# Tomeu7/AO-MARL

Measured on AMD Instinct MI355X. Metric: env steps/sec (AO frames/sec), higher is better.
Workload: dtype f32

## Files before the change

### ao_marl_amd/csrc/aomarl_capi.hip

```cpp
#include "aomarl_kernels.hip"

#include <math.h>
#include <stdlib.h>
#include <stdarg.h>
#include <stdio.h>
#include <string.h>

#include <algorithm>
#include <climits>
#include <string>
#include <vector>

static thread_local char g_err[512] = "";

int fail(const char *fmt, ...) {
  va_list ap;
  va_start(ap, fmt);
  vsnprintf(g_err, sizeof(g_err), fmt, ap);
  va_end(ap);
  return 1;
}


struct aomarl_ctx {
// ... 19 lines not shown
  bool small_ok = false;
  int reset_streams = 2;
  bool reset_prefetch_whole = true;
  hipEvent_t ev_reset = nullptr, ev_reset2[3] = {nullptr, nullptr, nullptr};
  bool no_extrude_sg = false;
  bool defer_dm_shape = false;
  int fused_debug = 0;
  bool prefetch_atmos = false, premoved = false;
  bool frame_wait_pending = false;
  bool screens_dirty_main = true;
  float cmat_scale = 1.f, v2m_scale = 1.f, m2v_scale = 1.f, s2m_scale = 1.f, ab_scale[AOMARL_MAX_LAYERS] = {1.f, 1.f, 1.f, 1.f, 1.f, 1.f, 1.f, 1.f};
  bool subpixel_flow = false;
  float frac_x[AOMARL_MAX_LAYERS] = {0, 0, 0, 0, 0, 0, 0, 0}, frac_y[AOMARL_MAX_LAYERS] = {0, 0, 0, 0, 0, 0, 0, 0};
  bool graph_step = false, capturing = false, side_joined = false, fork_recorded = false;
  hipEvent_t ev_fork = nullptr;
  struct StepGraph { std::vector<long long> key; hipGraphExec_t exec; hipGraph_t graph; unsigned long long arith[AR_N]; int fw_variant[6]; };
  std::vector<StepGraph> graphs;
  unsigned long long graph_hits = 0, graph_captures = 0;
  unsigned long long cfg_epoch = 0;
  const int32_t *sel_checked = nullptr;
  int sel_checked_n = 0, sel_checked_nm = 0;
  int fw_variant[6] = {0, 0, 0, 0, 0, 0};
  char fw_name[96] = {0};
  bool time_fw = false;
  std::vector<hipEvent_t> fw_ev;
  size_t fw_ev_used = 0;
  std::vector<hipEvent_t> fw_ev_retired;
  hipStream_t atm_stream = nullptr, psf_stream = nullptr;
  hipEvent_t ev_frame = nullptr, ev_moved = nullptr, ev_psf = nullptr;
  hipEvent_t ev_frame_cur = nullptr;
  bool frame_marked = false;
  struct FramePipe {
    bool have_twin = false, active = false;
    const float *owner_screens = nullptr;
    aomarl_state twin;
    int par = 0;
    hipStream_t fstream = nullptr;
    hipEvent_t ev_cmd = nullptr, ev_commit = nullptr, ev_done[2] = {nullptr, nullptr}, ev_psf[2] = {nullptr, nullptr};
    hipEvent_t ev_done_cur[2] = {nullptr, nullptr};
    bool psf_out[2] = {false, false};
    bool cmd_covers_commit = false;
    bool cmd_covers_psf = false;
    int32_t *snap[2] = {nullptr, nullptr};
    size_t snap_ints = 0;
    unsigned long long steps = 0, overlapped = 0, behind = 0;
  } pipe;
// ... 737 lines not shown
```

### ao_marl_amd/csrc/aomarl_capi_composites.hip

```cpp
const char *aomarl_frame_kernel_name(aomarl_ctx *c) {
  if (!c || !c->fw_variant[0]) return "";
  snprintf(c->fw_name, sizeof(c->fw_name), "k_frame_wave<%d, %d, %s, %s, %s, %s>", c->fw_variant[0], c->fw_variant[1],
           c->fw_variant[2] ? "true" : "false", c->fw_variant[3] ? "true" : "false",
           c->fw_variant[4] ? "true" : "false", c->fw_variant[5] ? "true" : "false");
  return c->fw_name;
}

int aomarl_frame_kernel_time(aomarl_ctx *c, double *total_ms, int *launches) {
  if (!c || !total_ms || !launches) return fail("frame_kernel_time: null argument");
  double tot = 0.0;
  int n = 0;
  for (size_t i = 0; i + 1 < c->fw_ev_used; i += 2) {
    float ms = 0.f;
    HIPCHK(hipEventSynchronize(c->fw_ev[i + 1]));
    HIPCHK(hipEventElapsedTime(&ms, c->fw_ev[i], c->fw_ev[i + 1]));
    tot += ms; n++;
  }
  { const int rrc = fw_ev_rewind(c); if (rrc) return rrc; }
  *total_ms = tot; *launches = n;
  return 0;
}

int aomarl_frame_fused_available(aomarl_ctx *c) {
  return c && c->sys.fused_ok && !c->force_unfused_frame ? 1 : 0;
}

static int frame_fused_impl(aomarl_ctx *c, aomarl_state *st, int b, int n, int flags, void *stream, int slot);

int aomarl_frame_fused(aomarl_ctx *c, aomarl_state *st, int b, int n, int flags, void *stream) {
  return frame_fused_impl(c, st, b, n, flags, stream, -1);
}

static int frame_fused_impl(aomarl_ctx *c, aomarl_state *st, int b, int n, int flags, void *stream, int slot) {
  int rc = check_range(c, st, b, n);
  if (rc) return rc;
  if (slot < 0) {
    rc = atmos_wait_pending(c, stream);
    if (rc) return rc;
    rc = psf_wait_pending(c, stream);
    if (rc) return rc;
  }
  if (!c->sys.fused_ok) return fail("frame_fused: geometry not eligible (see aomarl_frame_fused_available)");
  if (flags & (AOMARL_IMG_FROM_PHASE_BUFFER | AOMARL_IMG_NO_ATMOS | AOMARL_IMG_NO_DMS))
    return fail("frame_fused: FROM_PHASE_BUFFER / NO_ATMOS / NO_DMS are not supported here");
  const bool noise = (flags & AOMARL_IMG_NOISE) && c->sys.noise >= 0.f;
  const bool cube = flags & AOMARL_IMG_WRITE_BINCUBE;
  const bool otf = flags & AOMARL_IMG_DM_FROM_VOLTAGE;
  const int cog = ((flags & AOMARL_IMG_COG) ? 1 : 0) | (c->fused_debug << 8);
  if (otf && !c->sys.otf_ok) return fail("frame_fused: DM_FROM_VOLTAGE needs a separable stack-array lattice (see aomarl_dm_from_voltage_available)");
  if (cube && !st->bincube) return fail("frame_fused: WRITE_BINCUBE needs st->bincube");
  if (!cube && !(cog & 1)) return fail("frame_fused: nothing to produce (neither bincube nor slopes)");
  if (n == 0) return 0;
  hipStream_t s = (hipStream_t)stream;
  Work w = work_layout(c, st->nenv);
  const int W = 2 * c->sys.hw;
  float *TR = st->work + w.TR + (size_t)b * c->sys.pupdiam * W * 2;
  float *TP = st->work + w.TPART + (size_t)b * w.nblk * 4;
  float *PEND = st->work + w.PEND + (size_t)b * (W * W + 4);
  DevState ds = dev_state(st);
  if (w.nblk != c->sys.ntiles) return fail("frame_fused: internal stripe count mismatch");
  const int nb = otf ? c->sys.otf_nb : 1;
  const bool hp = c->dft_mode < 0 ? g_precision != 0 : c->dft_mode == 1;
  const bool qf = FW_QF && otf && !hp && !noise && !cube;
  const bool dma = FW_DMA && otf && (hp || FW_DMA_F32);
  const size_t smm = sizeof(float) * ((qf ? 0 : 2 * 128) + (otf ? 4 * 4 * nb * c->sys.otf_latw : 0)) + FW_SLOT_BYTES(dma) +
                     (dma ? 4 * FWD_WAVE(c->nlayers == 1 ? 1 : 3) : 128) +
                     (qf ? 4 * 16 * (size_t)c->sys.ntiles : 0);
  static const long lds_pad_env = [] { const char *e = getenv("AOMARL_FW_LDS_PAD"); return e ? atol(e) : -1L; }();
  size_t lds_pad = 0;
  if (qf && slot >= 0 && smm >= 40 * 1024) {
    const size_t two_per_cu = (160 * 1024) / 3 + 64;
    lds_pad = lds_pad_env >= 0 ? (size_t)lds_pad_env : (smm < two_per_cu ? (two_per_cu - smm + 63) / 64 * 64 : 0);
    if (smm + lds_pad > 64 * 1024) lds_pad = 0;
  }
  dim3 grid((n + 3) / 4, c->sys.ntiles), blk(256);
#define FW(NL, NB, OTF, NZ, WC, HP) hipExtLaunchKernelGGL((k_frame_wave<NL, NB, OTF, NZ, WC, HP>), grid, blk, smm + lds_pad, s, ev_start, ev_done, 0, c->sys, ds, b, n, cog, TR, TP, w.nblk)
#define FW_H(NL, NB, OTF, NZ, WC) do { if (hp) FW(NL, NB, OTF, NZ, WC, true); else FW(NL, NB, OTF, NZ, WC, false); } while (0)
#define FW_NC(NL, NB, OTF)                                                                     \
  do {                                                                                          \
    if (noise) { if (cube) FW_H(NL, NB, OTF, true, true); else FW_H(NL, NB, OTF, true, false); }     \
    else { if (cube) FW_H(NL, NB, OTF, false, true); else FW_H(NL, NB, OTF, false, false); }         \
  } while (0)
#define FW_L(NL)                                                          \
  do {                                                                    \
    if (!otf) FW_NC(NL, 1, false);                                        \
    else if (nb == 1) FW_NC(NL, 1, true);                                 \
    else FW_NC(NL, 2, true);                                              \
  } while (0)
  const bool timed = !c->capturing && c->time_fw && c->fw_ev_used + 2 <= c->fw_ev.size();
  hipEvent_t ev_start = nullptr, ev_done = nullptr;
  if (c->prefetch_atmos) {
    rc = side_stream(c);
    if (rc) return rc;
    ev_done = slot < 0 ? c->ev_frame : c->pipe.ev_done[slot];
  }
  if (timed) { ev_start = c->fw_ev[c->fw_ev_used]; ev_done = c->fw_ev[c->fw_ev_used + 1]; c->fw_ev_used += 2; }
  hipEvent_t ev_mark = nullptr;
  if (c->capturing) { ev_mark = ev_done; ev_start = nullptr; ev_done = nullptr; }
// ... 198 lines not shown
```

### ao_marl_amd/csrc/aomarl_capi_stages.hip

```cpp
static int dm_shape_impl(aomarl_ctx *c, aomarl_state *st, int b, int n, const float *volts,
                         bool skip_stack, void *stream) {
  const float *v = volts ? volts : st->voltage + (size_t)b * st->ld_actu;
  const int ldv = volts ? c->sys.nactu : st->ld_actu;
  DevState ds = dev_state(st);
  for (int k = 0; k < c->ndm; k++) {
    const DevDm &D = c->sys.dms[k];
    const int np = D.dim * D.dim;
    if (D.type == AOMARL_DM_TT)
      hipLaunchKernelGGL(k_dm_shape, dim3(1, n), dim3(64), 0, (hipStream_t)stream, c->sys, ds, b, k, v, ldv);
    else if (skip_stack)
      continue;
    else if (D.sep && !c->force_generic_dm)
      hipLaunchKernelGGL(k_dm_shape_sep, dim3((D.dim + DMS_TX - 1) / DMS_TX, (D.dim + DMS_TY - 1) / DMS_TY, n),
                         dim3(256), 0, (hipStream_t)stream, c->sys, ds, b, k, v, ldv);
    else
      hipLaunchKernelGGL(k_dm_shape, dim3((np + 255) / 256, n), dim3(256), 0, (hipStream_t)stream, c->sys, ds, b, k, v, ldv);
    LAUNCHCHK();
  }
  return 0;
}

int aomarl_comp_dm_shape(aomarl_ctx *c, aomarl_state *st, int b, int n, const float *volts, void *stream) {
  int rc = check_range(c, st, b, n);
  if (rc) return rc;
// ... 52 lines not shown
  if (!strcmp(name, "residual_shortcut")) {
    if (value && (!c->s2m || c->s2m_nmodes < 1)) return fail("residual_shortcut: no v2m . cmat matrix (aomarl_set_slopes2modes)");
    c->residual_shortcut = value != 0;
    return 0;
  }
  if (!strcmp(name, "reset_streams")) { c->reset_streams = value < 1 ? 1 : (value > 4 ? 4 : value); return 0; }
  if (!strcmp(name, "reset_prefetch_whole")) { c->reset_prefetch_whole = value != 0; return 0; }
  if (!strcmp(name, "extrude_unfused")) { c->no_extrude_sg = value != 0; return 0; }
  if (!strcmp(name, "reset_untransposed")) { c->reset_untransposed = value != 0; return 0; }
  if (!strcmp(name, "time_frame_kernel")) {
    c->time_fw = value > 0;
    { const int rrc = fw_ev_rewind(c); if (rrc) return rrc; }
    while (c->fw_ev.size() < 2 * (size_t)std::max(value, 0)) {
      hipEvent_t e;
      HIPCHK(hipEventCreate(&e));
      c->fw_ev.push_back(e);
    }
    return 0;
  }
  if (!strcmp(name, "prefetch_atmos")) { c->prefetch_atmos = value != 0; return 0; }
  if (!strcmp(name, "subpixel_flow")) { c->subpixel_flow = value != 0; return 0; }
  if (!strcmp(name, "graph_step")) { c->graph_step = value != 0; return 0; }
  if (!strcmp(name, "fused_debug")) { c->fused_debug = value; return 0; }
  if (!strcmp(name, "force_f32_dft")) { c->dft_mode = value < 0 ? -1 : (value != 0 ? 0 : 1); return 0; }
  if (!strcmp(name, "force_unfused_frame")) { c->force_unfused_frame = value != 0; return 0; }
  if (!strcmp(name, "force_generic_spot")) { c->force_generic_spot = value != 0; return 0; }
  if (!strcmp(name, "force_generic_target")) { c->force_generic_target = value != 0; return 0; }
  return fail("set_option: unknown option %s", name);
}

static DevSys traced_sys(const aomarl_ctx *c) {
  DevSys sy = c->sys;
  if (c->subpixel_flow)
    for (int l = 0; l < c->nlayers; l++) {
      sy.layers[l].wxo += c->frac_x[l]; sy.layers[l].txo += c->frac_x[l];
      sy.layers[l].wyo += c->frac_y[l]; sy.layers[l].tyo += c->frac_y[l];
    }
  return sy;
}

int aomarl_raytrace_wfs(aomarl_ctx *c, aomarl_state *st, int b, int n, int flags, void *stream) {
  int rc = check_range(c, st, b, n);
  if (rc) return rc;
  rc = atmos_wait_pending(c, stream);
  if (rc) return rc;
  if (!st->wfs_phase) return fail("raytrace_wfs needs st->wfs_phase");
// ... 350 lines not shown
```

### ao_marl_amd/csrc/aomarl_kernels.hip

```cpp
#include "aomarl_host.h"
#include "aomarl_gemm_p.h"
#include <type_traits>

#define WAVE 64

typedef unsigned u32x4 __attribute__((ext_vector_type(4)));

__device__ __forceinline__ hx2 cvt_h2(float a, float b) {
  return __builtin_bit_cast(hx2, __builtin_amdgcn_cvt_pkrtz(a, b));
}
__device__ __forceinline__ float sub_lo(hx2 h, float a) {
  float r;
  asm("v_fma_mix_f32 %0, %1, -1.0, %2 op_sel_hi:[1,0,0]" : "=v"(r) : "v"(h), "v"(a));
  return r;
}
__device__ __forceinline__ float sub_hi(hx2 h, float a) {
  float r;
  asm("v_fma_mix_f32 %0, %1, -1.0, %2 op_sel:[1,0,0] op_sel_hi:[1,0,0]" : "=v"(r) : "v"(h), "v"(a));
  return r;
}

struct __attribute__((packed, aligned(4))) f4u { float v[4]; };
__device__ __forceinline__ void add4(float acc[4], const float *p) {
  const f4u t = *reinterpret_cast<const f4u *>(p);
// ... 2088 lines not shown
#endif
#define FW_SLOT_BYTES(dma) ((dma) ? (FW_SLOTS1 ? 2 * 3 * 1024 : 16384) : 16384)
#define FWD_BLK 1152
#define FWD_IMG (2 * 1024 + 128)
#define FWD_WAVE(nl) ((nl) * FWD_IMG)
__global__ __launch_bounds__(256) __attribute__((amdgpu_waves_per_eu(FW_WAVES, FW_WAVES)))
void k_frame_wave(DevSys sys, DevState st, int env_begin,
                                                    int env_count, int do_cog,
                                                    float *__restrict__ TR,
                                                    float *__restrict__ TPART, int nblk) {
  extern __shared__ float smem[];
  const int pd = sys.pupdiam, ntl = sys.ntiles;
  const int tid = threadIdx.x, lane = tid & 63, q = lane >> 4, c = lane & 15;
  const int wv = __builtin_amdgcn_readfirstlane(tid >> 6);
  constexpr bool QF = FW_QF && OTF && !HP && !NOISE && !WRITE_CUBE;
  constexpr bool DMA = FW_DMA && OTF && (HP || FW_DMA_F32);
  float2 *sTw = reinterpret_cast<float2 *>(smem);
  float *lat_all = reinterpret_cast<float *>(sTw + (QF ? 0 : 128));
  float4 *shb = reinterpret_cast<float4 *>(lat_all + 4 * 4 * NB * (OTF ? sys.otf_latw : 0));
  char *dimg = reinterpret_cast<char *>(shb) + FW_SLOT_BYTES(DMA) + (DMA ? wv * FWD_WAVE(NL) : 0);
  float4 *qmom = reinterpret_cast<float4 *>(reinterpret_cast<char *>(shb) + FW_SLOT_BYTES(DMA) + (DMA ? 4 * FWD_WAVE(NL) : 0)) + wv * ntl;
  const int dbg = do_cog >> 8;
  do_cog &= 1;
  const int r = sys.stripe_order[blockIdx.y];
  const int el = 4 * blockIdx.x + wv;
  if constexpr (!QF) {
    if (tid < 128) {
      float sn, cs;
      sincospif((float)tid * (1.0f / 64.0f), &sn, &cs);
      sTw[tid] = make_float2(cs, sn);
    }
    __syncthreads();
  }
  const bool active = el < env_count;
  const int e = env_begin + (active ? el : env_count - 1);
  float Cc[4] = {0.f, 0.f, 0.f, 0.f}, Ss[4] = {0.f, 0.f, 0.f, 0.f};
  if constexpr (!QF) {
#pragma unroll
    for (int s = 0; s < 4; s++) {
      const float2 w = sTw[((4 * q + s) * (2 * c + 1)) & 127];
      Cc[s] = w.x; Ss[s] = w.y;
    }
  }
  SpotTwH twh;
  if (HP) twh = spot_tw_h(Cc, Ss);
  SpotQf qfk;
  if constexpr (QF) {
    const float4 ka = reinterpret_cast<const float4 *>(sys.qf_tab)[2 * lane], kb = reinterpret_cast<const float4 *>(sys.qf_tab)[2 * lane + 1];
    qfk.Ml = f32x2{ka.x, ka.y}; qfk.Mh = f32x2{ka.z, ka.w};
    qfk.Sl = f32x2{kb.x, kb.y}; qfk.Sh = f32x2{kb.z, kb.w};
  }
  unsigned shstep;
  const int y = 16 * r + c;
  const char *layb[NL];
  __amdgpu_buffer_rsrc_t lrs[NL];
  unsigned lpxs[NL], ldim[NL], lvo[NL];
#pragma unroll
  for (int l = 0; l < NL; l++) {
    const DevLayer &L = sys.layers[l];
    layb[l] = reinterpret_cast<const char *>(st.screens + (long long)e * sys.screen_stride + L.screen_off);
    lrs[l] = __builtin_amdgcn_make_buffer_rsrc(const_cast<char *>(layb[l]), 0,
                                               4 * L.dim * (L.dim + RING_PAD), 0x00020000);
    ldim[l] = (unsigned)L.dim;
    int px = L.tox + st.origin[(e * sys.nlayers + l) * 2]; px -= (px >= L.dim) ? L.dim : 0;
    int py = L.toy + st.origin[(e * sys.nlayers + l) * 2 + 1]; py -= (py >= L.dim) ? L.dim : 0;
    lpxs[l] = (unsigned)px;
    unsigned pr = (unsigned)y + (unsigned)py; pr = min(pr, pr - ldim[l]);
    lvo[l] = 4u * (pr * (ldim[l] + RING_PAD) + 4u * (unsigned)q);
  }
  const DevDm &D0 = sys.dms[0], &D1 = sys.dms[1];
  const float *pzt = st.dm_shape + (long long)e * sys.shape_stride + D0.shape_off;
  const float *ttslot = st.dm_shape + (long long)e * sys.shape_stride + D1.shape_off;
  const float c0 = ttslot[0], c1 = ttslot[1];
  const int half = pd / 2;
  const unsigned pvo = 4u * ((unsigned)(y + D0.toy) * (unsigned)D0.dim + (unsigned)D0.tox + 4u * (unsigned)q);
  const unsigned tvo = 32u * ((unsigned)y * (unsigned)(pd >> 2) + (unsigned)q);
  const unsigned mvo = 2u * (unsigned)y * (unsigned)ntl;
  const char *pztb = reinterpret_cast<const char *>(pzt);
  const char *ttb = reinterpret_cast<const char *>(sys.tt_pk);
  const char *mkb = reinterpret_cast<const char *>(sys.tile_mask);
  const bool sh_tt = wv < 2;
  const void *shbase = sh_tt ? static_cast<const void *>(ttb) : (HP ? sys.psf_tw_h : sys.psf_tw_f);
  const __amdgpu_buffer_rsrc_t shrs = __builtin_amdgcn_make_buffer_rsrc(
      const_cast<void *>(shbase), 0, sh_tt ? 8 * pd * pd : ntl * 1024, 0x00020000);
  const unsigned shvo = sh_tt ? tvo + 16u * (unsigned)wv : 16u * (unsigned)lane;
  shstep = sh_tt ? 7u : 10u;
  float pivot;
  {
    float v = OTF ? ttslot[2] : pzt[(half + D0.toy) * D0.dim + half + D0.tox];
    const float2 f = reinterpret_cast<const float2 *>(D1.influ)[(half + D1.toy) * D1.dim + half + D1.tox];
    v += c0 * f.x + c1 * f.y;
#pragma unroll
    for (int l = 0; l < NL; l++) {
      const DevLayer &L = sys.layers[l];
      int py = L.toy + st.origin[(e * sys.nlayers + l) * 2 + 1]; py -= (py >= L.dim) ? L.dim : 0;
      unsigned pyc = (unsigned)(half + py); pyc = min(pyc, pyc - ldim[l]);
      unsigned pxc = (unsigned)half + lpxs[l]; pxc = min(pxc, pxc - ldim[l]);
      v += reinterpret_cast<const float *>(layb[l])[pyc * (ldim[l] + RING_PAD) + pxc];
    }
    pivot = v;
  }
  float Pxr[NB], Pyr[NB];
  const int jm = (c >> 2) + 4 * (c & 3);
  const bool jm_ok = jm < 4 * NB;
  const int latw = sys.otf_latw, tpn = sys.otf_tpn;
  float *lat = lat_all + wv * (4 * NB * latw);
  if (OTF) {
#pragma unroll
    for (int s = 0; s < NB; s++) {
      const int ax = sys.otf_xoff + c - D0.pitch * (q + 4 * s);
      const int ay = sys.otf_yoff + c - D0.pitch * (q + 4 * s);
      Pxr[s] = (ax >= 0 && ax < D0.ss) ? D0.prof[ax] : 0.f;
      Pyr[s] = (ay >= 0 && ay < D0.ss) ? D0.prof[ay] : 0.f;
    }
    const float *volt = st.voltage + (long long)e * st.ld_actu + D0.com_off;
    for (int i = 0; i < 4 * NB; i++) {
      const int gy = sys.otf_gy0 + r * tpn + i;
      for (int jj = lane; jj < latw; jj += 64) {
        const int gx = sys.otf_gx0 + jj;
        float v = 0.f;
        if (gx >= 0 && gx < D0.gw && gy >= 0 && gy < D0.gh) {
          const int a = D0.grid[gy * D0.gw + gx];
          if (a >= 0) v = volt[a];
        }
        lat[i * latw + jj] = v;
      }
    }
    __builtin_amdgcn_wave_barrier();
  }
  const float *latq = lat + (jm_ok ? jm : 0);
  const float wfs_il = sys.wfs_inv_lambda, tar_il = sys.tar_inv_lambda;
  const f32x4 Z4 = opaque_zero4();
  f32x4 PA = {0.f, 0.f, 0.f, 0.f}, PB = {0.f, 0.f, 0.f, 0.f};
  float R0r = 0.f, R0i = 0.f;
  float sd = 0.f, sd2 = 0.f, sm = 0.f;
  int nlit = 0;
  constexpr bool PK = OTF && !HP;
  const f32x4 NP4 = {-pivot, -pivot, -pivot, -pivot};
  const f32x2 c0c0 = {c0, c0}, c1c1 = {c1, c1};
  const f32x2 wil2 = {sys.wfs_inv_lambda, sys.wfs_inv_lambda}, til2 = {sys.tar_inv_lambda, sys.tar_inv_lambda};
  f32x2 sdp = {0.f, 0.f}, sd2p = {0.f, 0.f}, R0rp = {0.f, 0.f}, R0ip = {0.f, 0.f};
  int nfull = 0;

  const const_float_p cflux = (const_float_p)(unsigned long long)sys.flux;
  auto fetch = [&](int info, FrameRaw<NL, OTF> &raw) {
    const int t = (info >> 24) & 0x7F;
    {
      const f32x4 v4 = __builtin_bit_cast(f32x4, __builtin_amdgcn_raw_buffer_load_b128(shrs, shvo, (unsigned)t << shstep, 0));
#pragma unroll
      for (int j = 0; j < 4; j++) raw.SH.v[j] = v4[j];
    }
    raw.mrow = *reinterpret_cast<const uint16_t *>(mkb + 2u * (unsigned)t + mvo);
#pragma unroll
    for (int l = 0; l < NL; l++) {
      unsigned sx = 16u * (unsigned)t + lpxs[l]; sx -= (sx >= ldim[l]) ? ldim[l] : 0u;
      const f32x4 v4 = __builtin_bit_cast(f32x4, __builtin_amdgcn_raw_buffer_load_b128(lrs[l], lvo[l], 4u * sx, 0));
#pragma unroll
      for (int j = 0; j < 4; j++) raw.L[l][j] = v4[j];
    }
    if (!OTF) {
      const f4u p4 = *reinterpret_cast<const f4u *>(pztb + 64u * (unsigned)t + pvo);
#pragma unroll
      for (int j = 0; j < 4; j++) raw.P[OTF ? 0 : j] = p4.v[j];
    }
    raw.F = cflux[info & 0xFFFF];
// ... 133 lines not shown
        PA = mfma16(ar[0], csP.x, PA); PB = mfma16(ai[0], csP.x, PB);
        PA = mfma16(ar[1], csP.y, PA); PB = mfma16(ai[1], csP.y, PB);
        PA = mfma16(ar[2], csP.z, PA); PB = mfma16(ai[2], csP.z, PB);
        PA = mfma16(ar[3], csP.w, PA); PB = mfma16(ai[3], csP.w, PB);
      }
    }
    if ((info & FW_SUB) && !(dbg & 1)) {
      if (HP) {
        float v[2][2][2];
        spot_dft_h_v(twh, wr, wi, Z4, v);
        spot_finish_v<NOISE, WRITE_CUBE>(sys, st, e, info & 0xFFFF, lane, v, do_cog, flux_i);
      } else if (!NOISE && !WRITE_CUBE) {
        if constexpr (QF) {
          const float z = spot_qf_moments(qfk, wr, wi, Z4);
          if (c == 0 && q < 3) reinterpret_cast<float *>(qmom + t)[q] = z;
        } else if constexpr (PK) spot_cog_f32_pk(sys, st, e, info & 0xFFFF, lane, Cc, Ss, wr, wi, do_cog, Z4);
        else spot_cog_f32(sys, st, e, info & 0xFFFF, lane, Cc, Ss, wr, wi, do_cog, Z4);
      } else {
        spot_core<NOISE, WRITE_CUBE>(sys, st, e, info & 0xFFFF, lane, Cc, Ss, wr, wi, do_cog, flux_i, Z4);
      }
    }
  };

  if constexpr (DMA) {
    const std::integral_constant<int, 1> dm;
    const int np = sys.pair_count[r];
    const const_int_p pinfo = (const_int_p)(unsigned long long)(sys.pair_info + r * (2 * ((ntl + 1) / 2 + 2)));
    const int rr = lane >> 3, kk = (lane & 7) ^ rr;
    unsigned dvo[NL][2];
#pragma unroll
    for (int l = 0; l < NL; l++) {
      const DevLayer &L = sys.layers[l];
      int py = L.toy + st.origin[(e * sys.nlayers + l) * 2 + 1]; py -= (py >= L.dim) ? L.dim : 0;
#pragma unroll
      for (int b = 0; b < 2; b++) {
        unsigned pr = (unsigned)(16 * r + 8 * b + rr) + (unsigned)py; pr = min(pr, pr - ldim[l]);
        dvo[l][b] = 4u * (pr * (ldim[l] + RING_PAD)) + 16u * (unsigned)kk;
      }
    }
    const int bc = c >> 3, rc = c & 7;
    const char *rdp[2];
#pragma unroll
    for (int h = 0; h < 2; h++) rdp[h] = dimg + bc * FWD_BLK + 16 * (rc * 8 + ((4 * h + q) ^ rc));
    const unsigned dimg_lds = (unsigned)(unsigned long long)dimg;
    FrameRaw<NL, OTF> A, B;
    unsigned mrA, mrB;
    float fA, fB;
    const unsigned shb_lds = (unsigned)(unsigned long long)shb + 1024u * (unsigned)wv;
    auto dma16 = [&](unsigned vo, __amdgpu_buffer_rsrc_t rs, unsigned lds_addr, unsigned so) {
      unsigned keep;
      asm volatile("s_mov_b32 %0, m0\n\ts_mov_b32 m0, %3\n\ts_nop 0\n\tbuffer_load_dwordx4 %1, %2, %4 offen lds\n\ts_mov_b32 m0, %0"
                   : "=&s"(keep) : "v"(vo), "s"(rs), "s"(lds_addr), "s"(so) : "memory");
    };
    auto issue_shared = [&](int ia, int ib, int par) {
      const int ta = (ia >> 24) & 0x7F, tb = (ib >> 24) & 0x7F;
      if (FW_SLOTS1) {
        if (wv < 3) {
          dma16(shvo, shrs, shb_lds, (unsigned)ta << shstep);
          dma16(shvo, shrs, shb_lds + 3072u, (unsigned)tb << shstep);
        }
      } else {
        dma16(shvo, shrs, shb_lds + (unsigned)par * 8192u, (unsigned)ta << shstep);
        dma16(shvo, shrs, shb_lds + (unsigned)par * 8192u + 4096u, (unsigned)tb << shstep);
      }
    };
    auto issue = [&](int ia, int ib) {
      const int ta = (ia >> 24) & 0x7F, tb = (ib >> 24) & 0x7F;
      mrA = *reinterpret_cast<const uint16_t *>(mkb + 2u * (unsigned)ta + mvo);
      mrB = *reinterpret_cast<const uint16_t *>(mkb + 2u * (unsigned)tb + mvo);
      fA = cflux[ia & 0xFFFF];
      fB = cflux[ib & 0xFFFF];
#pragma unroll
      for (int l = 0; l < NL; l++) {
        unsigned sx = 16u * (unsigned)(ta & ~1) + lpxs[l]; sx -= (sx >= ldim[l]) ? ldim[l] : 0u;
        const unsigned so = 4u * sx;
#pragma unroll
        for (int b = 0; b < 2; b++) dma16(dvo[l][b], lrs[l], dimg_lds + l * FWD_IMG + b * FWD_BLK, so);
      }
    };
    int ia = pinfo[0], ib = pinfo[1];
    if (np > 0) { issue_shared(ia, ib, 0); issue(ia, ib); }
    for (int k = 0; k < np; k++) {
      const int ja = pinfo[2 * k + 2], jb = pinfo[2 * k + 3];
      asm volatile("s_waitcnt vmcnt(0)" ::: "memory");
#pragma unroll
      for (int l = 0; l < NL; l++) {
        const float4 va = *reinterpret_cast<const float4 *>(rdp[0] + l * FWD_IMG);
        const float4 vb = *reinterpret_cast<const float4 *>(rdp[1] + l * FWD_IMG);
        A.L[l][0] = va.x; A.L[l][1] = va.y; A.L[l][2] = va.z; A.L[l][3] = va.w;
        B.L[l][0] = vb.x; B.L[l][1] = vb.y; B.L[l][2] = vb.z; B.L[l][3] = vb.w;
      }
      A.mrow = mrA; A.F = fA; B.mrow = mrB; B.F = fB;
      asm volatile("s_waitcnt lgkmcnt(0)" ::: "memory");
      if (FW_SLOTS1) {
        if (k + 1 < np) issue(ja, jb);
        __syncthreads();
        float4 *slots = shb;
        {
          const float4 a0 = slots[lane], a1 = slots[64 + lane];
          A.CS = slots[128 + lane];
          A.T[0] = a0.x; A.T[1] = a0.y; A.T[2] = a0.z; A.T[3] = a0.w; A.T[4] = a1.x; A.T[5] = a1.y; A.T[6] = a1.z; A.T[7] = a1.w;
        }
        if (ia & FW_LIT) tile(ia, 0, A, A, dm, slots);
        {
          const float4 b0 = slots[192 + lane], b1 = slots[256 + lane];
          B.CS = slots[320 + lane];
          B.T[0] = b0.x; B.T[1] = b0.y; B.T[2] = b0.z; B.T[3] = b0.w; B.T[4] = b1.x; B.T[5] = b1.y; B.T[6] = b1.z; B.T[7] = b1.w;
        }
        asm volatile("s_waitcnt lgkmcnt(0)" ::: "memory");
        __syncthreads();
        if (k + 1 < np) issue_shared(ja, jb, 0);
        if (ib & FW_LIT) tile(ib, 0, B, B, dm, slots);
      } else {
        float4 *slots = shb + (k & 1) * 512;
        __syncthreads();
        if (k + 1 < np) { issue_shared(ja, jb, (k + 1) & 1); issue(ja, jb); }
        if (ia & FW_LIT) tile(ia, 0, A, A, dm, slots);
        if (ib & FW_LIT) tile(ib, 0, B, B, dm, slots + 256);
      }
      ia = ja; ib = jb;
    }
  } else {
  const std::integral_constant<int, 0> nd;
  const std::integral_constant<int, 2> nf;
  const int nl = sys.lit_count[r];
  const const_int_p linfo = (const_int_p)(unsigned long long)(sys.lit_info + r * (ntl + 8));
  {
    constexpr int D = FW_DEPTH;
    FrameRaw<NL, OTF> raw[D];
    int inf[D];
#pragma unroll
    for (int d = 0; d < D; d++) { inf[d] = linfo[d]; fetch(inf[d], raw[d]); }
    const int rem = nl % D, nfull = nl - rem;
    for (int k = 0; k < nfull; k += D) {
      int nx[D];
#pragma unroll
      for (int d = 0; d < D; d++) nx[d] = linfo[k + D + d];
#pragma unroll
      for (int d = 0; d < D; d++) tile(inf[d], nx[d], raw[d], raw[d], nd, nullptr);
#pragma unroll
      for (int d = 0; d < D; d++) inf[d] = nx[d];
    }
#pragma unroll
    for (int d = 0; d + 1 < D; d++)
      if (rem > d) tile(inf[d], inf[d], raw[d], raw[d], nf, nullptr);
  }
  }
  if (!active) return;
  if constexpr (QF) {
    if (do_cog && !(dbg & 1)) {
      for (int tt = lane; tt < ntl; tt += 64) {
        const int ti = sys.tile_info[r * ntl + tt];
        if (ti & FW_SUB) {
          const float4 m = qmom[tt];
          float sx, sy;
          qf_slopes(sys, m.x, m.z, m.y, sx, sy);
          float *sl = st.slopes + (long long)e * sys.nslope;
          sl[ti & 0xFFFF] = sx;
          sl[sys.nvalid + (ti & 0xFFFF)] = sy;
        }
      }
    }
  }
  if constexpr (PK) {
    R0r += R0rp.x + R0rp.y; R0i += R0ip.x + R0ip.y;
    sd += sdp.x + sdp.y; sd2 += sd2p.x + sd2p.y; sm += 4.f * (float)nfull;
  }
  R0r += __shfl_xor(R0r, 16); R0r += __shfl_xor(R0r, 32);
  R0i += __shfl_xor(R0i, 16); R0i += __shfl_xor(R0i, 32);
#pragma unroll
  for (int j = 0; j < 4; j++) {
    const float oa = dpp_f<0x128>(PA[j]), ob = dpp_f<0x128>(PB[j]);
    const float z0r = __shfl(R0r, 4 * q + j), z0i = __shfl(R0i, 4 * q + j);
    float rr, ri;
    int kxi;
    if (c < 8) { rr = PA[j] - ob; ri = PB[j] + oa; kxi = 7 - c; }
    else if (c < 15) { rr = oa + PB[j]; ri = ob - PA[j]; kxi = c + 1; }
    else { rr = z0r; ri = z0i; kxi = 8; }
    float2 *o = reinterpret_cast<float2 *>(TR) + ((long long)el * pd + (16 * r + 4 * q + j)) * 16 + kxi;
    *o = make_float2(rr, ri);
  }
  sd = wave_sum(sd); sd2 = wave_sum(sd2); sm = wave_sum(sm);
  if (lane == 0) {
    float *pp = TPART + ((long long)el * nblk + r) * 4;
    pp[0] = sd; pp[1] = sd2; pp[2] = sm; pp[3] = 0.f;
  }
}

__global__ __launch_bounds__(256) void k_cog(DevSys sys, DevState st, int env_begin) {
  const int lane = threadIdx.x & 63, wv = threadIdx.x >> 6;
  const int i = blockIdx.x * 4 + wv;
  const int e = env_begin + blockIdx.y;
  if (i >= sys.nvalid) return;
  const int np2 = sys.npix * sys.npix;
  const float *im = st.bincube + ((long long)e * sys.nvalid + i) * np2;
  float s0 = 0.f, sx = 0.f, sy = 0.f;
  for (int p = lane; p < np2; p += 64) {
    float val = im[p];
    int y = p / sys.npix, x = p - y * sys.npix;
    s0 += val; sx += val * (float)x; sy += val * (float)y;
  }
#pragma unroll
  for (int o = 32; o >= 1; o >>= 1) {
    s0 += __shfl_xor(s0, o); sx += __shfl_xor(sx, o); sy += __shfl_xor(sy, o);
  }
  if (lane == 0) {
    float *sl = st.slopes + (long long)e * sys.nslope;
    if (s0 != 0.f) {
// ... 773 lines not shown
```

Baseline: 554,000.

## Make fused frame kernel persistent with prologue prefetch of next work item

```diff
diff --git a/ao_marl_amd/csrc/aomarl_capi.hip b/ao_marl_amd/csrc/aomarl_capi.hip
--- a/ao_marl_amd/csrc/aomarl_capi.hip
+++ b/ao_marl_amd/csrc/aomarl_capi.hip
@@ -65,6 +65,11 @@
   int sel_checked_n = 0, sel_checked_nm = 0;
   int fw_variant[6] = {0, 0, 0, 0, 0, 0};
   char fw_name[96] = {0};
+  int frame_persistent = [] { const char *e = getenv("AOMARL_FW_PERSISTENT"); return e ? (atoi(e) != 0 ? 1 : 0) : 1; }();
+  int frame_persistent_grid = 0;
+  int fw_ncu = 0;
+  struct FwOcc { const void *fn; size_t lds; int per_cu; };
+  std::vector<FwOcc> fw_occ;
   bool time_fw = false;
   std::vector<hipEvent_t> fw_ev;
   size_t fw_ev_used = 0;
diff --git a/ao_marl_amd/csrc/aomarl_capi_composites.hip b/ao_marl_amd/csrc/aomarl_capi_composites.hip
--- a/ao_marl_amd/csrc/aomarl_capi_composites.hip
+++ b/ao_marl_amd/csrc/aomarl_capi_composites.hip
@@ -29,6 +29,22 @@
 
 int aomarl_frame_fused(aomarl_ctx *c, aomarl_state *st, int b, int n, int flags, void *stream) {
   return frame_fused_impl(c, st, b, n, flags, stream, -1);
+}
+
+static int fw_resident_workgroups(aomarl_ctx *c, const void *fn, size_t lds, int *G) {
+  if (!c->fw_ncu) {
+    int dev = 0;
+    HIPCHK(hipGetDevice(&dev));
+    HIPCHK(hipDeviceGetAttribute(&c->fw_ncu, hipDeviceAttributeMultiprocessorCount, dev));
+  }
+  for (const auto &o : c->fw_occ)
+    if (o.fn == fn && o.lds == lds) { *G = o.per_cu * c->fw_ncu; return 0; }
+  int per = 0;
+  HIPCHK(hipOccupancyMaxActiveBlocksPerMultiprocessor(&per, fn, 256, lds));
+  if (per < 1 || c->fw_ncu < 1) return fail("frame_fused: the occupancy query finds no room for a workgroup");
+  c->fw_occ.push_back({fn, lds, per});
+  *G = per * c->fw_ncu;
+  return 0;
 }
 
 static int frame_fused_impl(aomarl_ctx *c, aomarl_state *st, int b, int n, int flags, void *stream, int slot) {
@@ -74,6 +90,16 @@
     if (smm + lds_pad > 64 * 1024) lds_pad = 0;
   }
   dim3 grid((n + 3) / 4, c->sys.ntiles), blk(256);
+  if (qf && dma && nb == 1 && c->frame_persistent) {
+    const void *fn = c->nlayers == 1 ? (const void *)k_frame_wave<1, 1, true, false, false, false>
+                                     : (const void *)k_frame_wave<3, 1, true, false, false, false>;
+    int G = c->frame_persistent_grid;
+    if (G <= 0) {
+      rc = fw_resident_workgroups(c, fn, smm + lds_pad, &G);
+      if (rc) return rc;
+    }
+    if ((unsigned)G < grid.x * grid.y) grid = dim3((unsigned)G, 1);
+  }
 #define FW(NL, NB, OTF, NZ, WC, HP) hipExtLaunchKernelGGL((k_frame_wave<NL, NB, OTF, NZ, WC, HP>), grid, blk, smm + lds_pad, s, ev_start, ev_done, 0, c->sys, ds, b, n, cog, TR, TP, w.nblk)
 #define FW_H(NL, NB, OTF, NZ, WC) do { if (hp) FW(NL, NB, OTF, NZ, WC, true); else FW(NL, NB, OTF, NZ, WC, false); } while (0)
 #define FW_NC(NL, NB, OTF)                                                                     \
diff --git a/ao_marl_amd/csrc/aomarl_capi_stages.hip b/ao_marl_amd/csrc/aomarl_capi_stages.hip
--- a/ao_marl_amd/csrc/aomarl_capi_stages.hip
+++ b/ao_marl_amd/csrc/aomarl_capi_stages.hip
@@ -98,6 +98,8 @@
   if (!strcmp(name, "subpixel_flow")) { c->subpixel_flow = value != 0; return 0; }
   if (!strcmp(name, "graph_step")) { c->graph_step = value != 0; return 0; }
   if (!strcmp(name, "fused_debug")) { c->fused_debug = value; return 0; }
+  if (!strcmp(name, "frame_persistent")) { c->frame_persistent = value != 0; c->cfg_epoch++; return 0; }
+  if (!strcmp(name, "frame_persistent_grid")) { c->frame_persistent_grid = value > 0 ? value : 0; c->cfg_epoch++; return 0; }
   if (!strcmp(name, "force_f32_dft")) { c->dft_mode = value < 0 ? -1 : (value != 0 ? 0 : 1); return 0; }
   if (!strcmp(name, "force_unfused_frame")) { c->force_unfused_frame = value != 0; return 0; }
   if (!strcmp(name, "force_generic_spot")) { c->force_generic_spot = value != 0; return 0; }
diff --git a/ao_marl_amd/csrc/aomarl_kernels.hip b/ao_marl_amd/csrc/aomarl_kernels.hip
--- a/ao_marl_amd/csrc/aomarl_kernels.hip
+++ b/ao_marl_amd/csrc/aomarl_kernels.hip
@@ -2134,8 +2134,11 @@
   float4 *qmom = reinterpret_cast<float4 *>(reinterpret_cast<char *>(shb) + FW_SLOT_BYTES(DMA) + (DMA ? 4 * FWD_WAVE(NL) : 0)) + wv * ntl;
   const int dbg = do_cog >> 8;
   do_cog &= 1;
-  const int r = sys.stripe_order[blockIdx.y];
-  const int el = 4 * blockIdx.x + wv;
+  constexpr bool PERS = QF && DMA && NB == 1;
+  const unsigned ngrp = (unsigned)(env_count + 3) >> 2, nitems = ngrp * (unsigned)ntl;
+  const unsigned G = gridDim.x * gridDim.y, wgid = blockIdx.y * gridDim.x + blockIdx.x;
+  auto item_of = [&](unsigned round) { return round * G + ((round & 1u) ? G - 1u - wgid : wgid); };
+  if (wgid >= nitems) return;
   if constexpr (!QF) {
     if (tid < 128) {
       float sn, cs;
@@ -2144,8 +2147,9 @@
     }
     __syncthreads();
   }
-  const bool active = el < env_count;
-  const int e = env_begin + (active ? el : env_count - 1);
+  int r = 0;
+  int el = 0, e = 0;
+  bool active = false;
   float Cc[4] = {0.f, 0.f, 0.f, 0.f}, Ss[4] = {0.f, 0.f, 0.f, 0.f};
   if constexpr (!QF) {
 #pragma unroll
@@ -2163,55 +2167,26 @@
     qfk.Sl = f32x2{kb.x, kb.y}; qfk.Sh = f32x2{kb.z, kb.w};
   }
   unsigned shstep;
-  const int y = 16 * r + c;
   const char *layb[NL];
   __amdgpu_buffer_rsrc_t lrs[NL];
-  unsigned lpxs[NL], ldim[NL], lvo[NL];
-#pragma unroll
-  for (int l = 0; l < NL; l++) {
-    const DevLayer &L = sys.layers[l];
-    layb[l] = reinterpret_cast<const char *>(st.screens + (long long)e * sys.screen_stride + L.screen_off);
-    lrs[l] = __builtin_amdgcn_make_buffer_rsrc(const_cast<char *>(layb[l]), 0,
-                                               4 * L.dim * (L.dim + RING_PAD), 0x00020000);
-    ldim[l] = (unsigned)L.dim;
-    int px = L.tox + st.origin[(e * sys.nlayers + l) * 2]; px -= (px >= L.dim) ? L.dim : 0;
-    int py = L.toy + st.origin[(e * sys.nlayers + l) * 2 + 1]; py -= (py >= L.dim) ? L.dim : 0;
-    lpxs[l] = (unsigned)px;
-    unsigned pr = (unsigned)y + (unsigned)py; pr = min(pr, pr - ldim[l]);
-    lvo[l] = 4u * (pr * (ldim[l] + RING_PAD) + 4u * (unsigned)q);
-  }
+  unsigned lpxs[NL], lpys[NL], ldim[NL], lvo[NL];
+#pragma unroll
+  for (int l = 0; l < NL; l++) ldim[l] = (unsigned)sys.layers[l].dim;
   const DevDm &D0 = sys.dms[0], &D1 = sys.dms[1];
-  const float *pzt = st.dm_shape + (long long)e * sys.shape_stride + D0.shape_off;
-  const float *ttslot = st.dm_shape + (long long)e * sys.shape_stride + D1.shape_off;
-  const float c0 = ttslot[0], c1 = ttslot[1];
+  float c0 = 0.f, c1 = 0.f;
   const int half = pd / 2;
-  const unsigned pvo = 4u * ((unsigned)(y + D0.toy) * (unsigned)D0.dim + (unsigned)D0.tox + 4u * (unsigned)q);
-  const unsigned tvo = 32u * ((unsigned)y * (unsigned)(pd >> 2) + (unsigned)q);
-  const unsigned mvo = 2u * (unsigned)y * (unsigned)ntl;
-  const char *pztb = reinterpret_cast<const char *>(pzt);
+  unsigned pvo = 0, tvo = 0, mvo = 0;
+  const char *pztb = nullptr;
   const char *ttb = reinterpret_cast<const char *>(sys.tt_pk);
   const char *mkb = reinterpret_cast<const char *>(sys.tile_mask);
   const bool sh_tt = wv < 2;
   const void *shbase = sh_tt ? static_cast<const void *>(ttb) : (HP ? sys.psf_tw_h : sys.psf_tw_f);
   const __amdgpu_buffer_rsrc_t shrs = __builtin_amdgcn_make_buffer_rsrc(
       const_cast<void *>(shbase), 0, sh_tt ? 8 * pd * pd : ntl * 1024, 0x00020000);
-  const unsigned shvo = sh_tt ? tvo + 16u * (unsigned)wv : 16u * (unsigned)lane;
+  unsigned shvo = 0;
   shstep = sh_tt ? 7u : 10u;
-  float pivot;
-  {
-    float v = OTF ? ttslot[2] : pzt[(half + D0.toy) * D0.dim + half + D0.tox];
-    const float2 f = reinterpret_cast<const float2 *>(D1.influ)[(half + D1.toy) * D1.dim + half + D1.tox];
-    v += c0 * f.x + c1 * f.y;
-#pragma unroll
-    for (int l = 0; l < NL; l++) {
-      const DevLayer &L = sys.layers[l];
-      int py = L.toy + st.origin[(e * sys.nlayers + l) * 2 + 1]; py -= (py >= L.dim) ? L.dim : 0;
-      unsigned pyc = (unsigned)(half + py); pyc = min(pyc, pyc - ldim[l]);
-      unsigned pxc = (unsigned)half + lpxs[l]; pxc = min(pxc, pxc - ldim[l]);
-      v += reinterpret_cast<const float *>(layb[l])[pyc * (ldim[l] + RING_PAD) + pxc];
-    }
-    pivot = v;
-  }
+  float pivot = 0.f;
+  const float2 ttc = reinterpret_cast<const float2 *>(D1.influ)[(half + D1.toy) * D1.dim + half + D1.tox];
   float Pxr[NB], Pyr[NB];
   const int jm = (c >> 2) + 4 * (c & 3);
   const bool jm_ok = jm < 4 * NB;
@@ -2225,22 +2200,84 @@
       Pxr[s] = (ax >= 0 && ax < D0.ss) ? D0.prof[ax] : 0.f;
       Pyr[s] = (ay >= 0 && ay < D0.ss) ? D0.prof[ay] : 0.f;
     }
-    const float *volt = st.voltage + (long long)e * st.ld_actu + D0.com_off;
-    for (int i = 0; i < 4 * NB; i++) {
-      const int gy = sys.otf_gy0 + r * tpn + i;
-      for (int jj = lane; jj < latw; jj += 64) {
-        const int gx = sys.otf_gx0 + jj;
-        float v = 0.f;
-        if (gx >= 0 && gx < D0.gw && gy >= 0 && gy < D0.gh) {
-          const int a = D0.grid[gy * D0.gw + gx];
-          if (a >= 0) v = volt[a];
+  }
+  const float *latq = lat + (jm_ok ? jm : 0);
+  typedef const DevSys __attribute__((address_space(4))) *sys_cp;
+  typedef const DevLayer __attribute__((address_space(4))) &layer_cr;
+  sys_cp sp = (sys_cp)__builtin_amdgcn_kernarg_segment_ptr();
+  auto item_args = [&]() __attribute__((always_inline)) {
+    if constexpr (PERS) asm volatile("" : "+s"(sp));
+  };
+  struct Pro {
+    int r, el, e;
+    int ox[NL], oy[NL];
+    float c0, c1, t2, cp[NL];
+    int la[4 * NB];
+    float lv[4 * NB];
+  };
+  auto pro_hop1 = [&](unsigned idx, Pro &P) __attribute__((always_inline)) {
+    const unsigned sy = (unsigned)__builtin_amdgcn_readfirstlane((int)(idx / ngrp));
+    P.r = sp->stripe_order[sy];
+    P.el = 4 * (int)(idx - sy * ngrp) + wv;
+    P.e = env_begin + (P.el < env_count ? P.el : env_count - 1);
+    const const_int_p org = (const_int_p)(unsigned long long)(st.origin + (P.e * sp->nlayers) * 2);
+#pragma unroll
+    for (int l = 0; l < NL; l++) {
+      P.ox[l] = org[2 * l];
+      P.oy[l] = org[2 * l + 1];
+    }
+    const const_float_p ttslot = (const_float_p)(unsigned long long)(st.dm_shape + (long long)P.e * sp->shape_stride + sp->dms[1].shape_off);
+    P.c0 = ttslot[0]; P.c1 = ttslot[1];
+    if (OTF) P.t2 = ttslot[2];
+    else P.t2 = ((const_float_p)(unsigned long long)(st.dm_shape + (long long)P.e * sp->shape_stride + sp->dms[0].shape_off))[(half + sp->dms[0].toy) * sp->dms[0].dim + half + sp->dms[0].tox];
+    if (OTF) {
+      const int gx = sp->otf_gx0 + lane;
+#pragma unroll
+      for (int i = 0; i < 4 * NB; i++) {
+        const int gy = sp->otf_gy0 + P.r * tpn + i;
+        int a = -1;
+        if (lane < latw && gx >= 0 && gx < sp->dms[0].gw && gy >= 0 && gy < sp->dms[0].gh) a = sp->dms[0].grid[gy * sp->dms[0].gw + gx];
+        P.la[i] = a;
+      }
+    }
+  };
+  auto pro_hop2 = [&](Pro &P) __attribute__((always_inline)) {
+#pragma unroll
+    for (int l = 0; l < NL; l++) {
+      layer_cr L = sp->layers[l];
+      int px = L.tox + P.ox[l]; px -= (px >= L.dim) ? L.dim : 0;
+      int py = L.toy + P.oy[l]; py -= (py >= L.dim) ? L.dim : 0;
+      unsigned pyc = (unsigned)(half + py); pyc = min(pyc, pyc - ldim[l]);
+      unsigned pxc = (unsigned)half + (unsigned)px; pxc = min(pxc, pxc - ldim[l]);
+      P.cp[l] = ((const_float_p)(unsigned long long)(st.screens + (long long)P.e * sp->screen_stride + L.screen_off))[pyc * (ldim[l] + RING_PAD) + pxc];
+    }
+    if (OTF) {
+      const float *volt = st.voltage + (long long)P.e * st.ld_actu + sp->dms[0].com_off;
+#pragma unroll
+      for (int i = 0; i < 4 * NB; i++) P.lv[i] = P.la[i] >= 0 ? volt[P.la[i]] : 0.f;
+    }
+  };
+  auto pro_store = [&](const Pro &P) __attribute__((always_inline)) {
+    if (OTF) {
+#pragma unroll
+      for (int i = 0; i < 4 * NB; i++)
+        if (lane < latw) lat[i * latw + lane] = P.lv[i];
+      const float *volt = st.voltage + (long long)P.e * st.ld_actu + sp->dms[0].com_off;
+      for (int i = 0; i < 4 * NB; i++) {
+        const int gy = sp->otf_gy0 + P.r * tpn + i;
+        for (int jj = lane + 64; jj < latw; jj += 64) {
+          const int gx = sp->otf_gx0 + jj;
+          float v = 0.f;
+          if (gx >= 0 && gx < sp->dms[0].gw && gy >= 0 && gy < sp->dms[0].gh) {
+            const int a = sp->dms[0].grid[gy * sp->dms[0].gw + gx];
+            if (a >= 0) v = volt[a];
+          }
+          lat[i * latw + jj] = v;
         }
-        lat[i * latw + jj] = v;
-      }
-    }
-    __builtin_amdgcn_wave_barrier();
-  }
-  const float *latq = lat + (jm_ok ? jm : 0);
+      }
+      __builtin_amdgcn_wave_barrier();
+    }
+  };
   const float wfs_il = sys.wfs_inv_lambda, tar_il = sys.tar_inv_lambda;
   const f32x4 Z4 = opaque_zero4();
   f32x4 PA = {0.f, 0.f, 0.f, 0.f}, PB = {0.f, 0.f, 0.f, 0.f};
@@ -2248,11 +2285,43 @@
   float sd = 0.f, sd2 = 0.f, sm = 0.f;
   int nlit = 0;
   constexpr bool PK = OTF && !HP;
-  const f32x4 NP4 = {-pivot, -pivot, -pivot, -pivot};
-  const f32x2 c0c0 = {c0, c0}, c1c1 = {c1, c1};
+  f32x4 NP4 = {0.f, 0.f, 0.f, 0.f};
+  f32x2 c0c0 = {0.f, 0.f}, c1c1 = {0.f, 0.f};
   const f32x2 wil2 = {sys.wfs_inv_lambda, sys.wfs_inv_lambda}, til2 = {sys.tar_inv_lambda, sys.tar_inv_lambda};
   f32x2 sdp = {0.f, 0.f}, sd2p = {0.f, 0.f}, R0rp = {0.f, 0.f}, R0ip = {0.f, 0.f};
   int nfull = 0;
+  auto derive = [&](const Pro &P) __attribute__((always_inline)) {
+    r = P.r; el = P.el; e = P.e;
+    active = el < env_count;
+    const int y = 16 * r + c;
+#pragma unroll
+    for (int l = 0; l < NL; l++) {
+      layer_cr L = sp->layers[l];
+      layb[l] = reinterpret_cast<const char *>(st.screens + (long long)e * sp->screen_stride + L.screen_off);
+      lrs[l] = __builtin_amdgcn_make_buffer_rsrc(const_cast<char *>(layb[l]), 0,
+                                                 4 * L.dim * (L.dim + RING_PAD), 0x00020000);
+      int px = L.tox + P.ox[l]; px -= (px >= L.dim) ? L.dim : 0;
+      int py = L.toy + P.oy[l]; py -= (py >= L.dim) ? L.dim : 0;
+      lpxs[l] = (unsigned)px; lpys[l] = (unsigned)py;
+      unsigned pr = (unsigned)y + (unsigned)py; pr = min(pr, pr - ldim[l]);
+      lvo[l] = 4u * (pr * (ldim[l] + RING_PAD) + 4u * (unsigned)q);
+    }
+    c0 = P.c0; c1 = P.c1;
+    pztb = reinterpret_cast<const char *>(st.dm_shape + (long long)e * sp->shape_stride + sp->dms[0].shape_off);
+    pvo = 4u * ((unsigned)(y + sp->dms[0].toy) * (unsigned)sp->dms[0].dim + (unsigned)sp->dms[0].tox + 4u * (unsigned)q);
+    tvo = 32u * ((unsigned)y * (unsigned)(pd >> 2) + (unsigned)q);
+    mvo = 2u * (unsigned)y * (unsigned)ntl;
+    shvo = sh_tt ? tvo + 16u * (unsigned)wv : 16u * (unsigned)lane;
+    {
+      float v = P.t2;
+      v += c0 * ttc.x + c1 * ttc.y;
+#pragma unroll
+      for (int l = 0; l < NL; l++) v += P.cp[l];
+      pivot = v;
+    }
+    NP4 = f32x4{-pivot, -pivot, -pivot, -pivot};
+    c0c0 = f32x2{c0, c0}; c1c1 = f32x2{c1, c1};
+  };
 
   const const_float_p cflux = (const_float_p)(unsigned long long)sys.flux;
   auto fetch = [&](int info, FrameRaw<NL, OTF> &raw) {
@@ -2432,65 +2501,90 @@
     }
   };
 
+  const int rr = lane >> 3, kk = (lane & 7) ^ rr;
+  unsigned dvo[NL][2];
+  const int bc = c >> 3, rc = c & 7;
+  const char *rdp[2];
+#pragma unroll
+  for (int h = 0; h < 2; h++) rdp[h] = dimg + bc * FWD_BLK + 16 * (rc * 8 + ((4 * h + q) ^ rc));
+  const unsigned dimg_lds = (unsigned)(unsigned long long)dimg;
+  FrameRaw<NL, OTF> A, B;
+  unsigned mrA = 0, mrB = 0;
+  float fA = 0.f, fB = 0.f;
+  const unsigned shb_lds = (unsigned)(unsigned long long)shb + 1024u * (unsigned)wv;
+  auto dma16 = [&](unsigned vo, __amdgpu_buffer_rsrc_t rs, unsigned lds_addr, unsigned so) {
+    unsigned keep;
+    asm volatile("s_mov_b32 %0, m0\n\ts_mov_b32 m0, %3\n\ts_nop 0\n\tbuffer_load_dwordx4 %1, %2, %4 offen lds\n\ts_mov_b32 m0, %0"
+                 : "=&s"(keep) : "v"(vo), "s"(rs), "s"(lds_addr), "s"(so) : "memory");
+  };
+  auto issue_shared = [&](int ia, int ib, int par) {
+    const int ta = (ia >> 24) & 0x7F, tb = (ib >> 24) & 0x7F;
+    if (FW_SLOTS1) {
+      if (wv < 3) {
+        dma16(shvo, shrs, shb_lds, (unsigned)ta << shstep);
+        dma16(shvo, shrs, shb_lds + 3072u, (unsigned)tb << shstep);
+      }
+    } else {
+      dma16(shvo, shrs, shb_lds + (unsigned)par * 8192u, (unsigned)ta << shstep);
+      dma16(shvo, shrs, shb_lds + (unsigned)par * 8192u + 4096u, (unsigned)tb << shstep);
+    }
+  };
+  auto issue = [&](int ia, int ib) {
+    const int ta = (ia >> 24) & 0x7F, tb = (ib >> 24) & 0x7F;
+    mrA = *reinterpret_cast<const uint16_t *>(mkb + 2u * (unsigned)ta + mvo);
+    mrB = *reinterpret_cast<const uint16_t *>(mkb + 2u * (unsigned)tb + mvo);
+    fA = cflux[ia & 0xFFFF];
+    fB = cflux[ib & 0xFFFF];
+#pragma unroll
+    for (int l = 0; l < NL; l++) {
+      unsigned sx = 16u * (unsigned)(ta & ~1) + lpxs[l]; sx -= (sx >= ldim[l]) ? ldim[l] : 0u;
+      const unsigned so = 4u * sx;
+#pragma unroll
+      for (int b = 0; b < 2; b++) dma16(dvo[l][b], lrs[l], dimg_lds + l * FWD_IMG + b * FWD_BLK, so);
+    }
+  };
+  int pk = 0, np = 0, ia = 0, ib = 0;
+  const_int_p pinfo = nullptr;
+  auto first_pair = [&]() __attribute__((always_inline)) {
+    np = sp->pair_count[r];
+    pinfo = (const_int_p)(unsigned long long)(sp->pair_info + r * (2 * ((ntl + 1) / 2 + 2)));
+#pragma unroll
+    for (int l = 0; l < NL; l++) {
+#pragma unroll
+      for (int b = 0; b < 2; b++) {
+        unsigned pr = (unsigned)(16 * r + 8 * b + rr) + lpys[l]; pr = min(pr, pr - ldim[l]);
+        dvo[l][b] = 4u * (pr * (ldim[l] + RING_PAD)) + 16u * (unsigned)kk;
+      }
+    }
+    ia = pinfo[0]; ib = pinfo[1];
+    if (np > 0) { issue_shared(ia, ib, pk & 1); issue(ia, ib); }
+  };
+
+  Pro N;
+  pro_hop1(item_of(0), N);
+  pro_hop2(N);
+  pro_store(N);
+  derive(N);
+#ifdef FW_DBG_PRO2
+  {
+    asm volatile("" :: "v"(pivot), "v"(lvo[0]), "v"(N.lv[0]), "v"(c0), "v"(c1));
+    unsigned i2 = item_of(0);
+    asm volatile("" : "+s"(i2));
+    pro_hop1(i2, N);
+    pro_hop2(N);
+    pro_store(N);
+    derive(N);
+  }
+#endif
+  if constexpr (DMA) first_pair();
+  for (unsigned round = 0;; round++) {
+    const unsigned nidx = item_of(round + 1);
+    const bool more = PERS && nidx < nitems;
+    item_args();
+    if (more) pro_hop1(nidx, N);
   if constexpr (DMA) {
     const std::integral_constant<int, 1> dm;
-    const int np = sys.pair_count[r];
-    const const_int_p pinfo = (const_int_p)(unsigned long long)(sys.pair_info + r * (2 * ((ntl + 1) / 2 + 2)));
-    const int rr = lane >> 3, kk = (lane & 7) ^ rr;
-    unsigned dvo[NL][2];
-#pragma unroll
-    for (int l = 0; l < NL; l++) {
-      const DevLayer &L = sys.layers[l];
-      int py = L.toy + st.origin[(e * sys.nlayers + l) * 2 + 1]; py -= (py >= L.dim) ? L.dim : 0;
-#pragma unroll
-      for (int b = 0; b < 2; b++) {
-        unsigned pr = (unsigned)(16 * r + 8 * b + rr) + (unsigned)py; pr = min(pr, pr - ldim[l]);
-        dvo[l][b] = 4u * (pr * (ldim[l] + RING_PAD)) + 16u * (unsigned)kk;
-      }
-    }
-    const int bc = c >> 3, rc = c & 7;
-    const char *rdp[2];
-#pragma unroll
-    for (int h = 0; h < 2; h++) rdp[h] = dimg + bc * FWD_BLK + 16 * (rc * 8 + ((4 * h + q) ^ rc));
-    const unsigned dimg_lds = (unsigned)(unsigned long long)dimg;
-    FrameRaw<NL, OTF> A, B;
-    unsigned mrA, mrB;
-    float fA, fB;
-    const unsigned shb_lds = (unsigned)(unsigned long long)shb + 1024u * (unsigned)wv;
-    auto dma16 = [&](unsigned vo, __amdgpu_buffer_rsrc_t rs, unsigned lds_addr, unsigned so) {
-      unsigned keep;
-      asm volatile("s_mov_b32 %0, m0\n\ts_mov_b32 m0, %3\n\ts_nop 0\n\tbuffer_load_dwordx4 %1, %2, %4 offen lds\n\ts_mov_b32 m0, %0"
-                   : "=&s"(keep) : "v"(vo), "s"(rs), "s"(lds_addr), "s"(so) : "memory");
-    };
-    auto issue_shared = [&](int ia, int ib, int par) {
-      const int ta = (ia >> 24) & 0x7F, tb = (ib >> 24) & 0x7F;
-      if (FW_SLOTS1) {
-        if (wv < 3) {
-          dma16(shvo, shrs, shb_lds, (unsigned)ta << shstep);
-          dma16(shvo, shrs, shb_lds + 3072u, (unsigned)tb << shstep);
-        }
-      } else {
-        dma16(shvo, shrs, shb_lds + (unsigned)par * 8192u, (unsigned)ta << shstep);
-        dma16(shvo, shrs, shb_lds + (unsigned)par * 8192u + 4096u, (unsigned)tb << shstep);
-      }
-    };
-    auto issue = [&](int ia, int ib) {
-      const int ta = (ia >> 24) & 0x7F, tb = (ib >> 24) & 0x7F;
-      mrA = *reinterpret_cast<const uint16_t *>(mkb + 2u * (unsigned)ta + mvo);
-      mrB = *reinterpret_cast<const uint16_t *>(mkb + 2u * (unsigned)tb + mvo);
-      fA = cflux[ia & 0xFFFF];
-      fB = cflux[ib & 0xFFFF];
-#pragma unroll
-      for (int l = 0; l < NL; l++) {
-        unsigned sx = 16u * (unsigned)(ta & ~1) + lpxs[l]; sx -= (sx >= ldim[l]) ? ldim[l] : 0u;
-        const unsigned so = 4u * sx;
-#pragma unroll
-        for (int b = 0; b < 2; b++) dma16(dvo[l][b], lrs[l], dimg_lds + l * FWD_IMG + b * FWD_BLK, so);
-      }
-    };
-    int ia = pinfo[0], ib = pinfo[1];
-    if (np > 0) { issue_shared(ia, ib, 0); issue(ia, ib); }
-    for (int k = 0; k < np; k++) {
+    for (int k = 0; k < np; k++, pk++) {
       const int ja = pinfo[2 * k + 2], jb = pinfo[2 * k + 3];
       asm volatile("s_waitcnt vmcnt(0)" ::: "memory");
 #pragma unroll
@@ -2502,6 +2596,7 @@
       }
       A.mrow = mrA; A.F = fA; B.mrow = mrB; B.F = fB;
       asm volatile("s_waitcnt lgkmcnt(0)" ::: "memory");
+      if (more && k == 0) pro_hop2(N);
       if (FW_SLOTS1) {
         if (k + 1 < np) issue(ja, jb);
         __syncthreads();
@@ -2522,14 +2617,15 @@
         if (k + 1 < np) issue_shared(ja, jb, 0);
         if (ib & FW_LIT) tile(ib, 0, B, B, dm, slots);
       } else {
-        float4 *slots = shb + (k & 1) * 512;
+        float4 *slots = shb + (pk & 1) * 512;
         __syncthreads();
-        if (k + 1 < np) { issue_shared(ja, jb, (k + 1) & 1); issue(ja, jb); }
+        if (k + 1 < np) { issue_shared(ja, jb, (pk + 1) & 1); issue(ja, jb); }
         if (ia & FW_LIT) tile(ia, 0, A, A, dm, slots);
         if (ib & FW_LIT) tile(ib, 0, B, B, dm, slots + 256);
       }
       ia = ja; ib = jb;
     }
+    if (more && np == 0) pro_hop2(N);
   } else {
   const std::integral_constant<int, 0> nd;
   const std::integral_constant<int, 2> nf;
@@ -2556,16 +2652,24 @@
       if (rem > d) tile(inf[d], inf[d], raw[d], raw[d], nf, nullptr);
   }
   }
-  if (!active) return;
+  const int r0 = r, el0 = el, e0 = e;
+  const bool act0 = active;
+  if (more) {
+    item_args();
+    pro_store(N);
+    derive(N);
+    if constexpr (DMA) first_pair();
+  }
+  if (act0) {
   if constexpr (QF) {
     if (do_cog && !(dbg & 1)) {
       for (int tt = lane; tt < ntl; tt += 64) {
-        const int ti = sys.tile_info[r * ntl + tt];
+        const int ti = sys.tile_info[r0 * ntl + tt];
         if (ti & FW_SUB) {
           const float4 m = qmom[tt];
           float sx, sy;
           qf_slopes(sys, m.x, m.z, m.y, sx, sy);
-          float *sl = st.slopes + (long long)e * sys.nslope;
+          float *sl = st.slopes + (long long)e0 * sys.nslope;
           sl[ti & 0xFFFF] = sx;
           sl[sys.nvalid + (ti & 0xFFFF)] = sy;
         }
@@ -2582,18 +2686,25 @@
   for (int j = 0; j < 4; j++) {
     const float oa = dpp_f<0x128>(PA[j]), ob = dpp_f<0x128>(PB[j]);
     const float z0r = __shfl(R0r, 4 * q + j), z0i = __shfl(R0i, 4 * q + j);
-    float rr, ri;
+    float rr_, ri;
     int kxi;
-    if (c < 8) { rr = PA[j] - ob; ri = PB[j] + oa; kxi = 7 - c; }
-    else if (c < 15) { rr = oa + PB[j]; ri = ob - PA[j]; kxi = c + 1; }
-    else { rr = z0r; ri = z0i; kxi = 8; }
-    float2 *o = reinterpret_cast<float2 *>(TR) + ((long long)el * pd + (16 * r + 4 * q + j)) * 16 + kxi;
-    *o = make_float2(rr, ri);
+    if (c < 8) { rr_ = PA[j] - ob; ri = PB[j] + oa; kxi = 7 - c; }
+    else if (c < 15) { rr_ = oa + PB[j]; ri = ob - PA[j]; kxi = c + 1; }
+    else { rr_ = z0r; ri = z0i; kxi = 8; }
+    float2 *o = reinterpret_cast<float2 *>(TR) + ((long long)el0 * pd + (16 * r0 + 4 * q + j)) * 16 + kxi;
+    *o = make_float2(rr_, ri);
   }
   sd = wave_sum(sd); sd2 = wave_sum(sd2); sm = wave_sum(sm);
   if (lane == 0) {
-    float *pp = TPART + ((long long)el * nblk + r) * 4;
+    float *pp = TPART + ((long long)el0 * nblk + r0) * 4;
     pp[0] = sd; pp[1] = sd2; pp[2] = sm; pp[3] = 0.f;
+  }
+  }
+  if (!more) break;
+  PA = f32x4{0.f, 0.f, 0.f, 0.f}; PB = f32x4{0.f, 0.f, 0.f, 0.f};
+  R0r = 0.f; R0i = 0.f; sd = 0.f; sd2 = 0.f; sm = 0.f;
+  sdp = f32x2{0.f, 0.f}; sd2p = f32x2{0.f, 0.f}; R0rp = f32x2{0.f, 0.f}; R0ip = f32x2{0.f, 0.f};
+  nfull = 0;
   }
 }
 
```

New measurement: 502,900. 0.908x the previous value.
